# zerohd4869/MM-DFN

Measured on AMD Instinct MI355X. Metric: utterances/sec (fwd+bwd), IEMOCAP-shaped batch, higher is better.
Workload: dtype f32; 1 GPU; cfg2 (BASELINE configs[1]): B=16 dialogues/GPU, L=110, dims 100/100/512, 2 GCN layers, P=2, dropout 0.50; utterances_per_gpu=1760, parallelism=dp1

## Files before the change

mm_dfn_amd/csrc/gemm_tn.hip:

```cpp
#include "mmdfn_internal.h"
#include "../../include/mmdfn_hip.h"
#include <stdlib.h>
#include <algorithm>
#include <stdint.h>

namespace {

constexpr int BR = 32;
constexpr int TM = 64, TN = 64;
constexpr int TNW = 112;
constexpr int LDA = TM + 4;
constexpr int LDB = TN + 4;
constexpr int BS_FLOATS = 32 * (TNW + 4);

inline bool tn_wide(int N) {
    const double e64 = (double)N / (64.0 * ((N + 63) / 64)), e112 = (double)N / (112.0 * ((N + 111) / 112));
    return e112 > e64 + 0.02;
}

template <bool WIDE>
__device__ __forceinline__ void gemm_tn_body(float (*As)[BR * LDA], float* Bs0, const float* __restrict__ A,
                                             const float* __restrict__ B, float* __restrict__ part,
                                             float* __restrict__ colpart, int R, int M, int N, int lda, int ldb,
                                             int rows_per_split, int bshift, int tile, int split) {
// ... 405 lines not shown
            const int64_t idx = t >> 3;
            const bool live = idx < total + M && (idx < total || cs != nullptr);
            const float* src = idx < total ? part + idx : colpart + (idx - total);
            const int64_t sstride = idx < total ? total : M;
            float s = 0.f;
            if (live) {
                int k = sub;
                for (; k + 56 < splits; k += 64) {
                    float v[8];
#pragma unroll
                    for (int e = 0; e < 8; ++e) v[e] = src[(int64_t)(k + 8 * e) * sstride];
#pragma unroll
                    for (int e = 0; e < 8; ++e) s += v[e];
                }
                for (; k < splits; k += 8) s += src[(int64_t)k * sstride];
            }
            s += __shfl_xor(s, 1, 64);
            s += __shfl_xor(s, 2, 64);
            s += __shfl_xor(s, 4, 64);
            if (live && sub == 0) {
                if (idx < total) {
                    const int m = (int)(idx / N);
                    float* dst = C + (int64_t)m * ldc + (idx - (int64_t)m * N);
                    *dst = acc ? *dst + s : s;
                } else {
                    const int m = (int)(idx - total);
                    cs[m] = acc ? cs[m] + s : s;
                    if (cs2 != nullptr) cs2[m] = acc ? cs2[m] + s : s;
                }
            }
        }
        return;
    }
    for (int64_t idx = (blockIdx.x - oq.blk_prefix[p]) * (int64_t)blockDim.x + threadIdx.x; idx < total + M; idx += stride) {
        if (idx < total) {
            float s = 0.f;
            int k = 0;
            for (; k + 8 <= splits; k += 8) {
                float v[8];
#pragma unroll
                for (int e = 0; e < 8; ++e) v[e] = part[(int64_t)(k + e) * total + idx];
#pragma unroll
                for (int e = 0; e < 8; ++e) s += v[e];
            }
            for (; k < splits; ++k) s += part[(int64_t)k * total + idx];
            const int m = (int)(idx / N);
            float* dst = C + (int64_t)m * ldc + (idx - (int64_t)m * N);
            *dst = acc ? *dst + s : s;
        } else if (cs != nullptr) {
            const int m = (int)(idx - total);
            float s = 0.f;
#pragma unroll 8
            for (int k = 0; k < splits; ++k) s += colpart[(int64_t)k * M + m];
            cs[m] = acc ? cs[m] + s : s;
            if (cs2 != nullptr) cs2[m] = acc ? cs2[m] + s : s;
        }
    }
}

}

static int tn_splits_for(int R, int M, int N, int rows_target) {
#ifdef MMDFN_TUNING
    if (const char* e = getenv("MMDFN_TN_SPLITS")) {
        const int v = atoi(e);
        if (v > 0) return v;
// ... 150 lines not shown
}
static int tall_eff_splits(int R, int M, const TallPlan& plan, int* rps_out) {
    const int target = M > 128 ? plan.rows7 : plan.rows2;
    int splits = (R + target - 1) / (target > 0 ? target : 1);
    if (splits < 1) splits = 1;
    const int rps = ((R + splits - 1) / splits + TBR - 1) / TBR * TBR;
    if (rps_out) *rps_out = rps;
    return (R + rps - 1) / rps;
}

static int batch_eff_splits(int R, int M, int N, int rows_target, int* rps_out) {
    int splits = tn_splits_for(R, M, N, 1000);
    if (rows_target > 1000) {
        splits = (R + rows_target - 1) / rows_target;
        if (splits < 1) splits = 1;
    }
    const int rps = ((R + splits - 1) / splits + BR - 1) / BR * BR;
    if (rps_out) *rps_out = rps;
    return (R + rps - 1) / rps;
}

#ifdef MMDFN_TUNING
static bool tns_enabled() { const char* e = getenv("MMDFN_TN_SPLIT"); return !e || atoi(e) != 0; }
#else
constexpr bool tns_enabled() { return true; }
#endif
static bool tns_wide(int N) {
#ifdef MMDFN_TUNING
    if (const char* e = getenv("MMDFN_TNS_WIDE")) { if (atoi(e) == 0) return false; }
#endif
    const int nn = (N + MMDFN_TNS_TN - 1) / MMDFN_TNS_TN, nw = (N + 2 * MMDFN_TNS_TN - 1) / (2 * MMDFN_TNS_TN);
    return 3 * nw < 2 * nn;
}
static int tns_tiles(int M, int N, int* nblocks, int* wide = nullptr) {
    const bool w = tns_wide(N);
    const int bw = w ? 2 * MMDFN_TNS_TN : MMDFN_TNS_TN;
    const int nb = (N + bw - 1) / bw;
    if (nblocks) *nblocks = nb;
    if (wide) *wide = w ? 1 : 0;
    return ((M + MMDFN_TNS_TM - 1) / MMDFN_TNS_TM) * nb;
}
static int tns_rows_target(int nseg, const int* R, const int* out, int nout, const int* M, const int* N, bool riders = false) {
    double units = 0.0;
    for (int s = 0; s < nseg; ++s) {
        const int o = out[s];
        if (o < 0 || o >= nout) continue;
        int wd = 0;
        const int tiles = tns_tiles(M[o], N[o], nullptr, &wd);
        units += (wd ? 1.5 : 1.0) * tiles * R[s];
    }
    double wgs = 384.0;
    if (riders) wgs = 160.0;
#ifdef MMDFN_TUNING
    if (const char* e = getenv("MMDFN_TNS_WGS")) wgs = atof(e);
    if (riders) { if (const char* e = getenv("MMDFN_RIDER_WGS")) wgs = atof(e); }
#endif
    int rt = (int)(units / wgs);
    rt = rt < 256 ? 256 : (rt > 4096 ? 4096 : rt);
    return rt;
}
static int tns_eff_splits(int R, int rows_target, int* rps_out) {
    int splits = 8 * ((R + 4 * rows_target) / (8 * rows_target));
    if (splits < 8) splits = 8;
    const int max_s = (R + 2 * MMDFN_TNS_BK - 1) / (2 * MMDFN_TNS_BK);
    if (splits > max_s) splits = max_s;
    if (splits < 1) splits = 1;
    const int rps = ((R + splits - 1) / splits + MMDFN_TNS_BK - 1) / MMDFN_TNS_BK * MMDFN_TNS_BK;
    if (rps_out) *rps_out = rps;
    return (R + rps - 1) / rps;
}

extern "C" int64_t mmdfn_gemm_tn_batch_workspace(int nseg, const int* R, const int* out, int nout, const int* M,
                                                 const int* N) {
    int64_t total = 0;
    const TallPlan plan = tall_plan(nseg, R, out, nout, M, N);
    const int rt = batch_rows_target(nseg, R, out, nout, M, N, plan.on);
    const int rt_split = tns_rows_target(nseg, R, out, nout, M, N);
    for (int s = 0; s < nseg; ++s) {
        const int o = out[s];
        if (o < 0 || o >= nout) return -1;
        int eff = batch_eff_splits(R[s], M[o], N[o], rt, nullptr);
        if (plan.on && tn_tall_shape1(R[s], M[o], N[o])) eff = std::max(eff, tall_eff_splits(R[s], M[o], plan, nullptr));
        eff = std::max(eff, tns_eff_splits(R[s], rt_split, nullptr));
        total += (int64_t)eff * ((int64_t)M[o] * N[o] + M[o]);
    }
    return total;
}

struct TnExt {
    int n;
    const float* const* part;
    const float* const* colpart;
    float* const* C;
    float* const* colsum;
    const int *M, *N, *ldc, *splits, *accumulate;
};
// ... 149 lines not shown
        std::stable_sort(ord, ord + nseg, [&](int a, int b) { return wg_len(a) > wg_len(b); });
        TnSplitSegs tq;
        tq.n = nseg;
        tq.wg_prefix[0] = 0;
        for (int k = 0; k < nseg; ++k) {
            const int s = ord[k], o = out[s];
            int nb = 1, wd = 0;
            const int tiles = tns_tiles(M[o], N[o], &nb, &wd);
            tq.wide[k] = wd;
            tq.A[k] = A[s]; tq.B[k] = B[s];
            tq.part[k] = part_base[o] + (int64_t)used[o] * M[o] * N[o];
            tq.colpart[k] = (oq.colsum[o] != nullptr) ? col_base[o] + (int64_t)used[o] * M[o] : nullptr;
            used[o] += seg_eff[s];
            tq.R[k] = R[s]; tq.lda[k] = lda[s]; tq.ldb[k] = ldb[s]; tq.bshift[k] = bshift ? bshift[s] : 0;
            tq.rows_per_split[k] = seg_rps[s]; tq.splits[k] = seg_eff[s]; tq.tiles[k] = tiles; tq.nblocks[k] = nb;
            tq.M[k] = M[o]; tq.N[k] = N[o];
            tq.wg_prefix[k + 1] = tq.wg_prefix[k] + tiles * 8 * ((seg_eff[s] + 7) / 8);
        }
        for (int k = nseg; k < MMDFN_TNS_MAXSEG; ++k) {
            tq.A[k] = tq.B[k] = nullptr; tq.part[k] = tq.colpart[k] = nullptr;
            tq.R[k] = tq.lda[k] = tq.ldb[k] = tq.bshift[k] = tq.rows_per_split[k] = tq.splits[k] = tq.tiles[k] = tq.nblocks[k] = 0;
            tq.M[k] = tq.N[k] = 0; tq.wide[k] = 0;
            tq.wg_prefix[k + 1] = tq.wg_prefix[nseg];
        }
        if (stage && riders != nullptr && nseg <= MMDFN_RIDER_MAXSEG && !riders->rider.valid) {
            RiderPlan& p = riders->rider;
            p.tq = tq;
            std::copy(outs, outs + nout, p.outs);
            p.nout = nout;
            p.valid = true;
            return 0;
        }
        if (int e = mmdfn_launch_gemm_tn_split(tq, st)) return e;
        hipLaunchKernelGGL(gemm_tn_batch_reduce_kernel, dim3(oq.blk_prefix[ntot]), dim3(256), 0, st, oq);
        MMDFN_CHECK_LAUNCH();
        return 0;
    }
    const bool use_wide = !tn_no_wide();
    int order[TN_MAXSEG], no = 0, ntall = 0;
    for (int pass = 0; pass < 3; ++pass)
        for (int s = 0; s < nseg; ++s) {
            const int kind = !seg_tall[s] ? 2 : (tall_kind(M[out[s]]) == 7 ? 0 : 1);
            if (kind != pass) continue;
            order[no++] = s;
            if (seg_tall[s]) ++ntall;
        }
    size_t tall_lds = ntall > 0 ? (size_t)(2 * BR * LDA + 2 * BS_FLOATS) * sizeof(float) : 0;
    sq.n = nseg;
    sq.wg_prefix[0] = 0;
    for (int k = 0; k < nseg; ++k) {
        const int s = order[k];
        const int o = out[s];
        const bool wide = !seg_tall[s] && use_wide && tn_wide(N[o]);
        const int tnw = wide ? TNW : TN;
        const int tiles = seg_tall[s] ? tall_blocks(N[o]) : ((M[o] + TM - 1) / TM) * ((N[o] + tnw - 1) / tnw);
        sq.wide[k] = seg_tall[s] ? tall_block_width(N[o]) : (wide ? 1 : 0);
        sq.A[k] = A[s]; sq.B[k] = B[s];
        sq.part[k] = part_base[o] + (int64_t)used[o] * M[o] * N[o];
        sq.colpart[k] = (oq.colsum[o] != nullptr) ? col_base[o] + (int64_t)used[o] * M[o] : nullptr;
        used[o] += seg_eff[s];
        sq.R[k] = R[s]; sq.lda[k] = lda[s]; sq.ldb[k] = ldb[s]; sq.bshift[k] = bshift ? bshift[s] : 0;
        sq.rows_per_split[k] = seg_rps[s]; sq.tiles[k] = tiles; sq.M[k] = M[o]; sq.N[k] = N[o];
        sq.wg_prefix[k + 1] = sq.wg_prefix[k] + tiles * seg_eff[s];
        if (seg_tall[s]) {
            const int bw = tall_block_width(N[o]);
            const size_t need = 2 * (size_t)(((TBR * M[o] * 4 + 1023) & ~1023) + ((TBR * bw * 4 + 1023) & ~1023)) + 1024;
// ... 89 lines not shown
```

mm_dfn_amd/csrc/gemm_tn_split.hip:

```cpp
#include "gemm_tn_split_body.h"
#include <stdlib.h>


namespace {

using namespace tnsb;

template <int ABL>
__global__ __launch_bounds__(512, 2) void gemm_tn_split_kernel(const TnSplitSegs sq, float* __restrict__ trace) {
    extern __shared__ __attribute__((aligned(16))) unsigned char tns_smem[];
    tns_block<ABL>(sq, (int)blockIdx.x, tns_smem, trace);
}

}

int mmdfn_launch_gemm_tn_split(const TnSplitSegs& sq, hipStream_t s) {
    void (*kern)(const TnSplitSegs, float*) = gemm_tn_split_kernel<0>;
    float* trace = nullptr;
#ifdef MMDFN_TUNING
    if (const char* e = getenv("MMDFN_TRACE_PTR")) trace = reinterpret_cast<float*>(strtoull(e, nullptr, 0));
    if (const char* e = getenv("MMDFN_TNS_ABL")) {
        switch (atoi(e)) {
            case 1: kern = gemm_tn_split_kernel<1>; break;
            case 2: kern = gemm_tn_split_kernel<2>; break;
            case 4: kern = gemm_tn_split_kernel<4>; break;
            case 7: kern = gemm_tn_split_kernel<7>; break;
            case 8: kern = gemm_tn_split_kernel<8>; break;
            case 15: kern = gemm_tn_split_kernel<15>; break;
            case 16: kern = gemm_tn_split_kernel<16>; break;
            default: break;
        }
    }
#endif
    if (int e = mmdfn_allow_big_lds(kern)) return e;
    hipLaunchKernelGGL(kern, dim3(sq.wg_prefix[sq.n]), dim3(512), LDS_B, s, sq, trace);
    MMDFN_CHECK_LAUNCH();
    return 0;
}
```

mm_dfn_amd/csrc/gemm_tn_split_body.h:

```cpp
#pragma once
#include "mmdfn_internal.h"
#include <type_traits>

namespace tnsb {

typedef __bf16 bf16x8 __attribute__((ext_vector_type(8)));
typedef uint32_t u32x4 __attribute__((ext_vector_type(4)));
typedef uint32_t u32x2 __attribute__((ext_vector_type(2)));
typedef short s16x4 __attribute__((ext_vector_type(4)));
#define LDS_AS(T, p) ((__attribute__((address_space(3))) T*)(p))

constexpr int SK = MMDFN_TNS_BK;
constexpr int TSM = MMDFN_TNS_TM;
constexpr int TSN = MMDFN_TNS_TN;
constexpr int NCT = TSN / 16;
constexpr int ROWB = 288;
constexpr int PLANE_B = SK * ROWB;
constexpr int IMG_B = 3 * PLANE_B;
constexpr int STAGE_B = 2 * IMG_B;
constexpr int LDS_B = 2 * STAGE_B;

__device__ __forceinline__ float as_f(uint32_t u) { return __builtin_bit_cast(float, u); }
__device__ __forceinline__ uint32_t as_u(float f) { return __builtin_bit_cast(uint32_t, f); }

__device__ __forceinline__ void cut4(float4 v, uint32_t himask, u32x2& p1, u32x2& p2, u32x2& p3) {
    float x0 = v.x, x1 = v.y, x2 = v.z, x3 = v.w;
    p1 = u32x2{__builtin_amdgcn_perm(as_u(x1), as_u(x0), 0x07060302u), __builtin_amdgcn_perm(as_u(x3), as_u(x2), 0x07060302u)};
    x0 -= as_f(as_u(x0) & himask); x1 -= as_f(as_u(x1) & himask); x2 -= as_f(as_u(x2) & himask); x3 -= as_f(as_u(x3) & himask);
    p2 = u32x2{__builtin_amdgcn_perm(as_u(x1), as_u(x0), 0x07060302u), __builtin_amdgcn_perm(as_u(x3), as_u(x2), 0x07060302u)};
    x0 -= as_f(as_u(x0) & himask); x1 -= as_f(as_u(x1) & himask); x2 -= as_f(as_u(x2) & himask); x3 -= as_f(as_u(x3) & himask);
    p3 = u32x2{__builtin_amdgcn_perm(as_u(x1), as_u(x0), 0x07060302u), __builtin_amdgcn_perm(as_u(x3), as_u(x2), 0x07060302u)};
}

__device__ __forceinline__ u32x4 tr_frag(uint32_t addr) {
    const s16x4 lo = __builtin_amdgcn_ds_read_tr16_b64_v4i16(LDS_AS(s16x4, (uintptr_t)addr));
    const s16x4 hi = __builtin_amdgcn_ds_read_tr16_b64_v4i16(LDS_AS(s16x4, (uintptr_t)(addr + 16 * ROWB)));
    const u32x2 l2 = __builtin_bit_cast(u32x2, lo), h2 = __builtin_bit_cast(u32x2, hi);
    return u32x4{l2.x, l2.y, h2.x, h2.y};
}

__device__ __forceinline__ f32x4 mfma16(u32x4 a, u32x4 b, f32x4 c) {
    return __builtin_amdgcn_mfma_f32_16x16x32_bf16(__builtin_bit_cast(bf16x8, a), __builtin_bit_cast(bf16x8, b), c, 0, 0, 0);
}

constexpr int WTN = 2 * MMDFN_TNS_TN;
constexpr int ROWB_W = 544;
constexpr int PLANE_W = SK * ROWB_W;
constexpr int IMG_W = 3 * PLANE_W;
static_assert(IMG_B + IMG_W <= LDS_B, "the wide form's single stage fits the narrow form's LDS");

__device__ __forceinline__ u32x4 tr_frag_w(uint32_t addr) {
    const s16x4 lo = __builtin_amdgcn_ds_read_tr16_b64_v4i16(LDS_AS(s16x4, (uintptr_t)addr));
    const s16x4 hi = __builtin_amdgcn_ds_read_tr16_b64_v4i16(LDS_AS(s16x4, (uintptr_t)(addr + 16 * ROWB_W)));
    const u32x2 l2 = __builtin_bit_cast(u32x2, lo), h2 = __builtin_bit_cast(u32x2, hi);
    return u32x4{l2.x, l2.y, h2.x, h2.y};
}

template <class SQ>
__device__ __forceinline__ void tns_wide_body(const SQ& sq, const int p, const int local, unsigned char* smem) {
    const int round = (local >> 3) / sq.tiles[p];
    const int tile = (local >> 3) - round * sq.tiles[p];
    const int split = 8 * round + (local & 7);
    if (split >= sq.splits[p]) return;
    const int nbn = sq.nblocks[p];
    const int bm = tile / nbn, bn = tile - bm * nbn;
    const int R = sq.R[p], M = sq.M[p], N = sq.N[p], lda = sq.lda[p], ldb = sq.ldb[p], bshift = sq.bshift[p];
    const float* __restrict__ A = sq.A[p];
    const float* __restrict__ B = sq.B[p];
    const int m0 = bm * TSM, n0 = bn * WTN;
    const int r_begin = split * sq.rows_per_split[p];
    const int r_end = min(R, r_begin + sq.rows_per_split[p]);
    const int nchunks = (r_end - r_begin + SK - 1) / SK;

    const int tid = threadIdx.x, lane = tid & 63;
    const int wv = __builtin_amdgcn_readfirstlane(tid >> 6);
    const int wr = wv & 3, wc = wv >> 2;
    const int quad = tid & 31, lrow = tid >> 5;
    const int qb = tid & 63, rb = tid >> 6;
    const int mrem = M - (m0 + 32 * wr);
    const int ntm = mrem <= 0 ? 0 : (mrem <= 16 ? 1 : 2);
    float* __restrict__ colpart = (bn == 0) ? sq.colpart[p] : nullptr;

    const int ca = (m0 + 4 * quad < M) ? m0 + 4 * quad : 0;
    const int cb = (qb < WTN / 4 && n0 + 4 * qb < N) ? n0 + 4 * qb : 0;
    const uint32_t lds0 = (uint32_t)(uintptr_t)((__attribute__((address_space(3))) void*)smem);
    const uint32_t wra = lds0 + lrow * ROWB + quad * 8;
    const uint32_t wrb = lds0 + IMG_B + rb * ROWB_W + qb * 8;
    const uint32_t rsel = 4 * (lane >> 4) + ((lane & 15) >> 2);
    const uint32_t rda = lds0 + rsel * ROWB + (lane & 3) * 8 + 64 * wr;
    const uint32_t rdb = lds0 + IMG_B + rsel * ROWB_W + (lane & 3) * 8 + 2 * MMDFN_TNS_TN * wc;
    uint32_t himask;
    asm volatile("s_mov_b32 %0, 0xffff0000" : "=s"(himask));

    f32x4 acc[2][NCT];
#pragma unroll
    for (int i = 0; i < 2; ++i)
#pragma unroll
        for (int j = 0; j < NCT; ++j) acc[i][j] = (f32x4){0.f, 0.f, 0.f, 0.f};
    float4 cs = make_float4(0.f, 0.f, 0.f, 0.f);
    float4 na[2], nb[4];

    auto inside = [&](int c) {
        const int r0 = r_begin + c * SK;
        return c < nchunks && r0 + SK <= r_end && r0 + bshift >= 0 && r0 + SK - 1 + bshift < R;
    };
    uint32_t offa[2], offb[4];
#pragma unroll
    for (int e = 0; e < 2; ++e) offa[e] = (uint32_t)((lrow + 16 * e) * lda + ca) << 2;
#pragma unroll
    for (int e = 0; e < 4; ++e) offb[e] = (uint32_t)((rb + 8 * e) * ldb + cb) << 2;
    auto issue = [&](int c) {
        uint32_t va[2], vb[4];
        if (inside(c)) {
            const int r0 = r_begin + c * SK;
            const uint32_t sa = (uint32_t)(r0 * lda) << 2, sb = (uint32_t)((r0 + bshift) * ldb) << 2;
#pragma unroll
            for (int e = 0; e < 2; ++e) va[e] = sa + offa[e];
#pragma unroll
            for (int e = 0; e < 4; ++e) vb[e] = sb + offb[e];
        } else {
            const int r0 = r_begin + (c < nchunks ? c : nchunks - 1) * SK;
#pragma unroll
            for (int e = 0; e < 2; ++e) {
                const int rc = min(r0 + lrow + 16 * e, r_end - 1);
                va[e] = (__umul24((uint32_t)rc, (uint32_t)lda) + (uint32_t)ca) << 2;
            }
#pragma unroll
            for (int e = 0; e < 4; ++e) {
                const int rc = min(r0 + rb + 8 * e, r_end - 1);
                const int rbc = min(max(rc + bshift, 0), R - 1);
                vb[e] = (__umul24((uint32_t)rbc, (uint32_t)ldb) + (uint32_t)cb) << 2;
            }
        }
#pragma unroll
        for (int e = 0; e < 2; ++e) na[e] = *reinterpret_cast<const float4*>(reinterpret_cast<const char*>(A) + va[e]);
#pragma unroll
        for (int e = 0; e < 4; ++e) nb[e] = *reinterpret_cast<const float4*>(reinterpret_cast<const char*>(B) + vb[e]);
    };
    float4 ta[2], tb[4];
    auto stage_body = [&](auto edge_tag, int c) {
        constexpr bool EDGE = decltype(edge_tag)::value;
        const int r0 = r_begin + c * SK;
#pragma unroll
        for (int e = 0; e < 2; ++e) {
            float4 xa = ta[e];
            if (EDGE) {
                const bool aok = r0 + lrow + 16 * e < r_end;
                xa = make_float4(aok ? xa.x : 0.f, aok ? xa.y : 0.f, aok ? xa.z : 0.f, aok ? xa.w : 0.f);
            }
            if (colpart) { cs.x += xa.x; cs.y += xa.y; cs.z += xa.z; cs.w += xa.w; }
            u32x2 a1, a2, a3;
            cut4(xa, himask, a1, a2, a3);
            const uint32_t d = wra + e * 16 * ROWB;
            *LDS_AS(u32x2, (uintptr_t)d) = a1;
            *LDS_AS(u32x2, (uintptr_t)(d + PLANE_B)) = a2;
            *LDS_AS(u32x2, (uintptr_t)(d + 2 * PLANE_B)) = a3;
        }
#pragma unroll
        for (int e = 0; e < 4; ++e) {
            float4 xb = tb[e];
            if (EDGE) {
                const int r = r0 + rb + 8 * e;
                const bool bok = r < r_end && r + bshift >= 0 && r + bshift < R;
                xb = make_float4(bok ? xb.x : 0.f, bok ? xb.y : 0.f, bok ? xb.z : 0.f, bok ? xb.w : 0.f);
            }
            u32x2 b1, b2, b3;
            cut4(xb, himask, b1, b2, b3);
            const uint32_t d = wrb + e * 8 * ROWB_W;
            *LDS_AS(u32x2, (uintptr_t)d) = b1;
            *LDS_AS(u32x2, (uintptr_t)(d + PLANE_W)) = b2;
            *LDS_AS(u32x2, (uintptr_t)(d + 2 * PLANE_W)) = b3;
        }
    };
    auto stage = [&](int c) {
#pragma unroll
        for (int e = 0; e < 2; ++e) ta[e] = na[e];
#pragma unroll
        for (int e = 0; e < 4; ++e) tb[e] = nb[e];
        __builtin_amdgcn_sched_barrier(0);
        issue(c + 1);
        __builtin_amdgcn_sched_barrier(0);
        if (inside(c)) stage_body(std::false_type{}, c);
        else stage_body(std::true_type{}, c);
    };
    const int ncol = N - (n0 + MMDFN_TNS_TN * wc);
    const int nlive = ncol <= 0 ? 0 : (ncol >= MMDFN_TNS_TN ? NCT : (ncol + 15) / 16);
    auto mma = [&](auto ntm_tag, auto nl_tag) {
        constexpr int NTM = decltype(ntm_tag)::value;
        constexpr int NL = decltype(nl_tag)::value;
        u32x4 af[NTM][3], bf[3][NL];
#pragma unroll
        for (int q = 0; q < 3; ++q)
#pragma unroll
            for (int i = 0; i < NTM; ++i) af[i][q] = tr_frag(rda + q * PLANE_B + 32 * i);
#pragma unroll
        for (int q = 0; q < 3; ++q)
#pragma unroll
            for (int j = 0; j < NL; ++j) bf[q][j] = tr_frag_w(rdb + q * PLANE_W + 32 * j);
#pragma unroll
        for (int pc = 0; pc < 6; ++pc) {
            const int ai = (pc == 0) ? 2 : (pc == 1 || pc == 3) ? 1 : 0;
            const int bi = (pc < 3) ? 0 : (pc < 5) ? 1 : 2;
#pragma unroll
            for (int j = 0; j < NL; ++j)
#pragma unroll
                for (int i = 0; i < NTM; ++i) acc[i][j] = mfma16(af[i][ai], bf[bi][j], acc[i][j]);
        }
    };
    auto mma_nl = [&](auto ntm_tag) {
        switch (nlive) {
            case 7: mma(ntm_tag, std::integral_constant<int, 7>{}); break;
            case 6: mma(ntm_tag, std::integral_constant<int, 6>{}); break;
            case 5: mma(ntm_tag, std::integral_constant<int, 5>{}); break;
            case 4: mma(ntm_tag, std::integral_constant<int, 4>{}); break;
            case 3: mma(ntm_tag, std::integral_constant<int, 3>{}); break;
            case 2: mma(ntm_tag, std::integral_constant<int, 2>{}); break;
            case 1: mma(ntm_tag, std::integral_constant<int, 1>{}); break;
            default: break;
        }
    };

    issue(0);
#pragma unroll 1
    for (int k = 0; k < nchunks; ++k) {
        stage(k);
        __syncthreads();
        if (ntm == 2) mma_nl(std::integral_constant<int, 2>{});
        else if (ntm == 1) mma_nl(std::integral_constant<int, 1>{});
        __syncthreads();
    }
    if (ntm > 0) {
        float* P = sq.part[p] + (int64_t)split * M * N;
        const int fi = lane & 15, g = lane >> 4;
#pragma unroll
        for (int i = 0; i < 2; ++i)
#pragma unroll
            for (int j = 0; j < NCT; ++j) {
                const int n = n0 + MMDFN_TNS_TN * wc + 16 * j + fi;
#pragma unroll
                for (int r = 0; r < 4; ++r) {
                    const int m = m0 + 32 * wr + 16 * i + 4 * g + r;
                    if (m < M && n < N) P[(int64_t)m * N + n] = acc[i][j][r];
                }
            }
    }
    if (colpart) {
        float* red = reinterpret_cast<float*>(smem);
        *reinterpret_cast<float4*>(red + (tid >> 5) * TSM + 4 * quad) = cs;
        __syncthreads();
        if (tid < TSM && m0 + tid < M) {
            float s = 0.f;
#pragma unroll
            for (int k = 0; k < 16; ++k) s += red[k * TSM + tid];
            colpart[(int64_t)split * M + m0 + tid] = s;
        }
    }
}

template <int ABL, class SQ>
__device__ __forceinline__ void tns_block(const SQ& sq, const int bid, unsigned char* tns_smem, float* __restrict__ trace) {
    int p = 0;
    while (p + 1 < sq.n && bid >= sq.wg_prefix[p + 1]) ++p;
    const int local = bid - sq.wg_prefix[p];
    if (sq.wide[p]) {
        if (ABL == 0) tns_wide_body(sq, p, local, tns_smem);
        return;
    }
    const int round = (local >> 3) / sq.tiles[p];
    const int tile = (local >> 3) - round * sq.tiles[p];
    const int split = 8 * round + (local & 7);
    if (split >= sq.splits[p]) return;
    const int nbn = sq.nblocks[p];
    const int bm = tile / nbn, bn = tile - bm * nbn;
    const int R = sq.R[p], M = sq.M[p], N = sq.N[p], lda = sq.lda[p], ldb = sq.ldb[p], bshift = sq.bshift[p];
    const float* __restrict__ A = sq.A[p];
    const float* __restrict__ B = sq.B[p];
    const int m0 = bm * TSM, n0 = bn * TSN;
    const int r_begin = split * sq.rows_per_split[p];
    const int r_end = min(R, r_begin + sq.rows_per_split[p]);
    const int nchunks = (r_end - r_begin + SK - 1) / SK;

    const int tid = threadIdx.x, lane = tid & 63;
    const int wv = __builtin_amdgcn_readfirstlane(tid >> 6);
    const int grp = wv >> 2, w = wv & 3;
    const int quad = tid & 31, lrow = (tid >> 5) & 7;
    const int mrem = M - (m0 + 32 * w);
    const int ntm = mrem <= 0 ? 0 : (mrem <= 16 ? 1 : 2);
    float* __restrict__ colpart = (bn == 0) ? sq.colpart[p] : nullptr;

    const int ca = (m0 + 4 * quad < M) ? m0 + 4 * quad : 0;
    const int cb = (quad < TSN / 4 && n0 + 4 * quad < N) ? n0 + 4 * quad : 0;
    const uint32_t lds0 = (uint32_t)(uintptr_t)((__attribute__((address_space(3))) void*)tns_smem) + grp * STAGE_B;
    const uint32_t wr = lds0 + lrow * ROWB + quad * 8;
    const uint32_t rd = lds0 + (4 * (lane >> 4) + ((lane & 15) >> 2)) * ROWB + (lane & 3) * 8;
    uint32_t himask;
    asm volatile("s_mov_b32 %0, 0xffff0000" : "=s"(himask));

    f32x4 acc[2][NCT];
// ... 120 lines not shown
            for (int i = 0; i < NTM; ++i)
#pragma unroll
                for (int j = 0; j < NCT; ++j)
                    acc[i][j][0] += as_f(af[i][0].x ^ af[i][1].y ^ af[i][2].z ^ bf[0][j].x ^ bf[1][j].y ^ bf[2][j].z);
            return;
        }
#pragma unroll
        for (int pc = 0; pc < 6; ++pc) {
            const int ai = (pc == 0) ? 2 : (pc == 1 || pc == 3) ? 1 : 0;
            const int bi = (pc < 3) ? 0 : (pc < 5) ? 1 : 2;
#pragma unroll
            for (int j = 0; j < NCT; ++j)
#pragma unroll
                for (int i = 0; i < NTM; ++i) acc[i][j] = mfma16(af[i][ai], bf[bi][j], acc[i][j]);
        }
    };

    issue(grp);
    if (grp == 0) stage(0);
    __syncthreads();
    const long long t_begin = now();
#pragma unroll 1
    for (int k = 0; k < nchunks; ++k) {
        if ((k & 1) == grp) {
            const long long t0 = now();
            if (ntm == 2) mma(std::integral_constant<int, 2>{});
            else if (ntm == 1) mma(std::integral_constant<int, 1>{});
            if (ABL & 16) asm volatile("s_nop 0" ::: "memory");
            tm[3] += now() - t0;
        } else if (k + 1 < nchunks) {
            stage(k + 1);
        }
        const long long t3 = now();
        __syncthreads();
        tm[4] += now() - t3;
    }
    if ((ABL & 16) && trace && (tid == 0 || tid == 256)) {
        float* o = trace + (int64_t)bid * 32 + (tid ? 16 : 0);
        o[0] = (float)tm[0]; o[1] = (float)tm[1]; o[2] = (float)tm[2]; o[3] = (float)tm[3]; o[4] = (float)tm[4];
        o[6] = (float)nchunks; o[7] = (float)(now() - t_begin);
    }
    if (grp == 1 && ntm > 0) {
        float* xch = reinterpret_cast<float*>(tns_smem + (LDS_B - 2 * NCT * 4096)) + (w * 64 + lane) * 4;
#pragma unroll
        for (int i = 0; i < 2; ++i)
#pragma unroll
            for (int j = 0; j < NCT; ++j) *reinterpret_cast<f32x4*>(xch + (i * NCT + j) * 1024) = acc[i][j];
    }
    __syncthreads();
    if (grp == 0 && ntm > 0) {
        const float* xch = reinterpret_cast<const float*>(tns_smem + (LDS_B - 2 * NCT * 4096)) + (w * 64 + lane) * 4;
#pragma unroll
        for (int i = 0; i < 2; ++i)
#pragma unroll
            for (int j = 0; j < NCT; ++j) acc[i][j] += *reinterpret_cast<const f32x4*>(xch + (i * NCT + j) * 1024);
        float* P = sq.part[p] + (int64_t)split * M * N;
        const int fi = lane & 15, g = lane >> 4;
#pragma unroll
        for (int i = 0; i < 2; ++i)
#pragma unroll
            for (int j = 0; j < NCT; ++j) {
                const int n = n0 + 16 * j + fi;
#pragma unroll
                for (int r = 0; r < 4; ++r) {
                    const int m = m0 + 32 * w + 16 * i + 4 * g + r;
                    if (m < M && n < N) P[(int64_t)m * N + n] = acc[i][j][r];
                }
            }
    }
    if (colpart) {
        float* red = reinterpret_cast<float*>(tns_smem);
        *reinterpret_cast<float4*>(red + (tid >> 5) * TSM + 4 * quad) = cs;
        __syncthreads();
        if (tid < TSM && m0 + tid < M) {
            float s = 0.f;
#pragma unroll
            for (int k = 0; k < 16; ++k) s += red[k * TSM + tid];
            colpart[(int64_t)split * M + m0 + tid] = s;
        }
    }
}
}
```

mm_dfn_amd/csrc/gru_mfma.hip:

```cpp
#include "mmdfn_internal.h"
#include "gemm_tn_split_body.h"
#include "keep_flags_body.h"
#include <stdlib.h>

namespace {

constexpr int GH = 100;
typedef __bf16 bf16x8 __attribute__((ext_vector_type(8)));
typedef uint32_t u32x4 __attribute__((ext_vector_type(4)));
typedef uint32_t u32x2 __attribute__((ext_vector_type(2)));
#define LDS_AS(T, p) ((__attribute__((address_space(3))) T*)(p))

constexpr int MS = 16;
constexpr int NWV = 7;
constexpr int NTH = 64 * NWV;
constexpr int HROWB = 272;
constexpr int HPLANE = MS * HROWB;
constexpr int DROWB = 656;
constexpr int DPLANE = MS * DROWB;

__device__ __forceinline__ float as_f(uint32_t u) { return __builtin_bit_cast(float, u); }
__device__ __forceinline__ uint32_t as_u(float f) { return __builtin_bit_cast(uint32_t, f); }

__device__ __forceinline__ void cut4(float x0, float x1, float x2, float x3, u32x2& p1, u32x2& p2, u32x2& p3) {
// ... 387 lines not shown
            u32x2 p1, p2, p3;
            cut4(drp[0], drp[1], drp[2], drp[3], p1, p2, p3);
            *LDS_AS(u32x2, (uintptr_t)wb) = p1;
            *LDS_AS(u32x2, (uintptr_t)(wb + DPLANE)) = p2;
            *LDS_AS(u32x2, (uintptr_t)(wb + 2 * DPLANE)) = p3;
            cut4(dzp[0], dzp[1], dzp[2], dzp[3], p1, p2, p3);
            *LDS_AS(u32x2, (uintptr_t)(wb + 2 * GH)) = p1;
            *LDS_AS(u32x2, (uintptr_t)(wb + 2 * GH + DPLANE)) = p2;
            *LDS_AS(u32x2, (uintptr_t)(wb + 2 * GH + 2 * DPLANE)) = p3;
            cut4(dgn[0], dgn[1], dgn[2], dgn[3], p1, p2, p3);
            *LDS_AS(u32x2, (uintptr_t)(wb + 4 * GH)) = p1;
            *LDS_AS(u32x2, (uintptr_t)(wb + 4 * GH + DPLANE)) = p2;
            *LDS_AS(u32x2, (uintptr_t)(wb + 4 * GH + 2 * DPLANE)) = p3;
        }
        step_barrier();
        if (uok && rok) {
            float* o = dgi + t * gstep;
            *reinterpret_cast<float4*>(o) = make_float4(drp[0], drp[1], drp[2], drp[3]);
            *reinterpret_cast<float4*>(o + GH) = make_float4(dzp[0], dzp[1], dzp[2], dzp[3]);
            *reinterpret_cast<float4*>(o + 2 * GH) = make_float4(dnp[0], dnp[1], dnp[2], dnp[3]);
            float* h = dgh + t * gstep;
            __builtin_nontemporal_store(f32x4{drp[0], drp[1], drp[2], drp[3]}, reinterpret_cast<f32x4*>(h));
            __builtin_nontemporal_store(f32x4{dzp[0], dzp[1], dzp[2], dzp[3]}, reinterpret_cast<f32x4*>(h + GH));
            __builtin_nontemporal_store(f32x4{dgn[0], dgn[1], dgn[2], dgn[3]}, reinterpret_cast<f32x4*>(h + 2 * GH));
        }
    }
}

__global__ __launch_bounds__(BWD_THREADS) void gru_seq_bwd_mfma_kernel(const MfBwd G) {
    extern __shared__ __attribute__((aligned(16))) unsigned char gm_smem[];
    gru_bwd_mfma_body(G, (int)blockIdx.x, (int)blockIdx.y, gm_smem);
}

static_assert(BWD_THREADS == 512 && BWD_LDS >= tnsb::LDS_B, "the rider tiles run in this launch's workgroup shape");
__global__ __launch_bounds__(BWD_THREADS) void gru_seq_bwd_mfma_riders_kernel(const MfBwd G, const TnRiderSegs rq, const int nslots,
                                                                               const int ngru8) {
    extern __shared__ __attribute__((aligned(16))) unsigned char gm_smem[];
    const int bid = (int)blockIdx.x;
    if (bid < 2 * nslots) {
        gru_bwd_mfma_body(G, bid % nslots, bid / nslots, gm_smem);
    } else if (bid >= ngru8) {
        tnsb::tns_block<0>(rq, bid - ngru8, gm_smem, nullptr);
    }
}

}

int mmdfn_launch_gru_fwd_mfma(const GruForm& f, int ngroups, const float* const* gi, const float* const* w_hh,
                              const float* const* b_hh, float* const* y, float* const* gates, const int* rows, const int* T,
                              MmdfnRiders* riders, hipStream_t s) {
    if (ngroups <= 0 || ngroups > MAXG) return -2;
    MfFwd G;
    G.n = ngroups;
    int sl = 0;
    for (int g = 0; g < MAXG; ++g) {
        const bool on = g < ngroups;
        G.gi[g] = on ? gi[g] : nullptr; G.y[g] = on ? y[g] : nullptr; G.gates[g] = on ? gates[g] : nullptr;
        G.w_hh[2 * g] = on ? w_hh[2 * g] : nullptr; G.w_hh[2 * g + 1] = on ? w_hh[2 * g + 1] : nullptr;
        G.b_hh[2 * g] = on ? b_hh[2 * g] : nullptr; G.b_hh[2 * g + 1] = on ? b_hh[2 * g + 1] : nullptr;
        G.rows[g] = on ? rows[g] : 0; G.T[g] = on ? T[g] : 0; G.slice0[g] = sl;
        if (on) sl += (rows[g] + MS - 1) / MS;
    }
    G.slice0[MAXG] = sl;
    for (int g = ngroups; g < MAXG; ++g) G.slice0[g] = sl;
    G.abl = 0;
#ifdef MMDFN_TUNING
    if (const char* e = getenv("MMDFN_GRU_MF_ABL")) G.abl = atoi(e);
// ... 7 lines not shown
        hipLaunchKernelGGL(gru_seq_fwd_mfma_flags_kernel, dim3(2 * sl + (int)nr), dim3(FWD_THREADS), FWD_LDS, s, G, J, sl);
        MMDFN_CHECK_LAUNCH();
        return 0;
    }
    if (int e = mmdfn_allow_big_lds(gru_seq_fwd_mfma_kernel)) return e;
    hipLaunchKernelGGL(gru_seq_fwd_mfma_kernel, dim3(sl, 2), dim3(FWD_THREADS), FWD_LDS, s, G);
    MMDFN_CHECK_LAUNCH();
    return 0;
}

int mmdfn_launch_gru_bwd_mfma(const GruForm& f, int ngroups, const float* const* dy, const float* const* y,
                              const float* const* gates, const float* const* w_hh, float* const* dgi, float* const* dgh,
                              const int* rows, const int* T, MmdfnRiders* riders, hipStream_t s) {
    if (ngroups <= 0 || ngroups > MAXG) return -2;
    MfBwd G;
    G.n = ngroups;
    int sl = 0;
    for (int g = 0; g < MAXG; ++g) {
        const bool on = g < ngroups;
        G.dy[g] = on ? dy[g] : nullptr; G.y[g] = on ? y[g] : nullptr; G.gates[g] = on ? gates[g] : nullptr;
        G.w_hh[2 * g] = on ? w_hh[2 * g] : nullptr; G.w_hh[2 * g + 1] = on ? w_hh[2 * g + 1] : nullptr;
        G.dgi[g] = on ? dgi[g] : nullptr; G.dgh[g] = on ? dgh[g] : nullptr;
        G.rows[g] = on ? rows[g] : 0; G.T[g] = on ? T[g] : 0; G.slice0[g] = sl;
        if (on) sl += (rows[g] + MS - 1) / MS;
    }
    G.slice0[MAXG] = sl;
    for (int g = ngroups; g < MAXG; ++g) G.slice0[g] = sl;
    G.abl = 0;
    if (f.idle_cus > 0 && riders != nullptr && riders->rider.valid && riders->rider.tq.n <= MMDFN_RIDER_MAXSEG) {
        const TnSplitSegs& rp = riders->rider.tq;
        const TnRiderSegs rq = mmdfn_rider_table(rp);
        const int ngru8 = (2 * sl + 7) & ~7;
        if (int e = mmdfn_allow_big_lds(gru_seq_bwd_mfma_riders_kernel)) return e;
        hipLaunchKernelGGL(gru_seq_bwd_mfma_riders_kernel, dim3(ngru8 + rp.wg_prefix[rp.n]), dim3(BWD_THREADS), BWD_LDS, s, G, rq, sl,
                           ngru8);
        MMDFN_CHECK_LAUNCH();
        return mmdfn_riders_launched(riders, s);
    }
    if (int e = mmdfn_allow_big_lds(gru_seq_bwd_mfma_kernel)) return e;
    hipLaunchKernelGGL(gru_seq_bwd_mfma_kernel, dim3(sl, 2), dim3(BWD_THREADS), BWD_LDS, s, G);
    MMDFN_CHECK_LAUNCH();
    return 0;
}
```

Measured before the change: 2.152 million utterances/s.

## Double-buffer wide split-K TN GEMM stages and vectorize the split reduction

The wide form of the split-K TN GEMM now keeps two LDS stages and alternates warp groups between staging the next chunk and running MFMA on the current one, so global loads and LDS writes overlap the products with one barrier per chunk. LDS_B grows to two wide stages, which also raises the rider launch's dynamic LDS. The split-partials reduce kernel gains a float4 path when N, ldc and pointers are 16-byte aligned. The change also adds tuning-only ablation templates and env knobs. The larger LDS footprint keeps one workgroup per CU and may affect the rider kernel co-running with the GRU backward.

```diff
diff --git a/mm_dfn_amd/csrc/gemm_tn.hip b/mm_dfn_amd/csrc/gemm_tn.hip
--- a/mm_dfn_amd/csrc/gemm_tn.hip
+++ b/mm_dfn_amd/csrc/gemm_tn.hip
@@ -461,6 +461,40 @@
         }
         return;
     }
+    if (((N | ldc) & 3) == 0 && ((((uintptr_t)part | (uintptr_t)C) & 15) == 0)) {
+        const int64_t tot4 = total >> 2;
+        for (int64_t idx = (blockIdx.x - oq.blk_prefix[p]) * (int64_t)blockDim.x + threadIdx.x; idx < tot4 + M; idx += stride) {
+            if (idx < tot4) {
+                const float4* src = reinterpret_cast<const float4*>(part) + idx;
+                float4 s = make_float4(0.f, 0.f, 0.f, 0.f);
+                int k = 0;
+                for (; k + 8 <= splits; k += 8) {
+                    float4 v[8];
+#pragma unroll
+                    for (int e = 0; e < 8; ++e) v[e] = src[(int64_t)(k + e) * tot4];
+#pragma unroll
+                    for (int e = 0; e < 8; ++e) { s.x += v[e].x; s.y += v[e].y; s.z += v[e].z; s.w += v[e].w; }
+                }
+                for (; k < splits; ++k) {
+                    const float4 v = src[(int64_t)k * tot4];
+                    s.x += v.x; s.y += v.y; s.z += v.z; s.w += v.w;
+                }
+                const int64_t e0 = idx << 2;
+                const int m = (int)(e0 / N);
+                float4* dst = reinterpret_cast<float4*>(C + (int64_t)m * ldc + (e0 - (int64_t)m * N));
+                if (acc) { const float4 c = *dst; s.x = c.x + s.x; s.y = c.y + s.y; s.z = c.z + s.z; s.w = c.w + s.w; }
+                *dst = s;
+            } else if (cs != nullptr) {
+                const int m = (int)(idx - tot4);
+                float s = 0.f;
+#pragma unroll 8
+                for (int k = 0; k < splits; ++k) s += colpart[(int64_t)k * M + m];
+                cs[m] = acc ? cs[m] + s : s;
+                if (cs2 != nullptr) cs2[m] = acc ? cs2[m] + s : s;
+            }
+        }
+        return;
+    }
     for (int64_t idx = (blockIdx.x - oq.blk_prefix[p]) * (int64_t)blockDim.x + threadIdx.x; idx < total + M; idx += stride) {
         if (idx < total) {
             float s = 0.f;
@@ -677,12 +711,18 @@
     const int nn = (N + MMDFN_TNS_TN - 1) / MMDFN_TNS_TN, nw = (N + 2 * MMDFN_TNS_TN - 1) / (2 * MMDFN_TNS_TN);
     return 3 * nw < 2 * nn;
 }
+static int tns_wide_form() {
+#ifdef MMDFN_TUNING
+    if (const char* e = getenv("MMDFN_TNS_WIDE")) { if (atoi(e) == 2) return 2; }
+#endif
+    return 1;
+}
 static int tns_tiles(int M, int N, int* nblocks, int* wide = nullptr) {
     const bool w = tns_wide(N);
     const int bw = w ? 2 * MMDFN_TNS_TN : MMDFN_TNS_TN;
     const int nb = (N + bw - 1) / bw;
     if (nblocks) *nblocks = nb;
-    if (wide) *wide = w ? 1 : 0;
+    if (wide) *wide = w ? tns_wide_form() : 0;
     return ((M + MMDFN_TNS_TM - 1) / MMDFN_TNS_TM) * nb;
 }
 static int tns_rows_target(int nseg, const int* R, const int* out, int nout, const int* M, const int* N, bool riders = false) {
@@ -705,8 +745,12 @@
     return rt;
 }
 static int tns_eff_splits(int R, int rows_target, int* rps_out) {
-    int splits = 8 * ((R + 4 * rows_target) / (8 * rows_target));
-    if (splits < 8) splits = 8;
+    int unit = 8;
+#ifdef MMDFN_TUNING
+    if (const char* e = getenv("MMDFN_TNS_SPLIT_UNIT")) { if (atoi(e) > 0) unit = atoi(e); }
+#endif
+    int splits = unit * ((R + unit * rows_target / 2) / (unit * rows_target));
+    if (splits < unit) splits = unit;
     const int max_s = (R + 2 * MMDFN_TNS_BK - 1) / (2 * MMDFN_TNS_BK);
     if (splits > max_s) splits = max_s;
     if (splits < 1) splits = 1;
@@ -922,6 +966,9 @@
             return 0;
         }
         if (int e = mmdfn_launch_gemm_tn_split(tq, st)) return e;
+#ifdef MMDFN_TUNING
+        if (const char* e = getenv("MMDFN_TNS_NOREDUCE")) { if (atoi(e) != 0) return 0; }
+#endif
         hipLaunchKernelGGL(gemm_tn_batch_reduce_kernel, dim3(oq.blk_prefix[ntot]), dim3(256), 0, st, oq);
         MMDFN_CHECK_LAUNCH();
         return 0;
diff --git a/mm_dfn_amd/csrc/gemm_tn_split.hip b/mm_dfn_amd/csrc/gemm_tn_split.hip
--- a/mm_dfn_amd/csrc/gemm_tn_split.hip
+++ b/mm_dfn_amd/csrc/gemm_tn_split.hip
@@ -28,6 +28,11 @@
             case 8: kern = gemm_tn_split_kernel<8>; break;
             case 15: kern = gemm_tn_split_kernel<15>; break;
             case 16: kern = gemm_tn_split_kernel<16>; break;
+            case 32: kern = gemm_tn_split_kernel<32>; break;
+            case 64: kern = gemm_tn_split_kernel<64>; break;
+            case 47: kern = gemm_tn_split_kernel<47>; break;
+            case 79: kern = gemm_tn_split_kernel<79>; break;
+            case 111: kern = gemm_tn_split_kernel<111>; break;
             default: break;
         }
     }
diff --git a/mm_dfn_amd/csrc/gemm_tn_split_body.h b/mm_dfn_amd/csrc/gemm_tn_split_body.h
--- a/mm_dfn_amd/csrc/gemm_tn_split_body.h
+++ b/mm_dfn_amd/csrc/gemm_tn_split_body.h
@@ -18,7 +18,7 @@
 constexpr int PLANE_B = SK * ROWB;
 constexpr int IMG_B = 3 * PLANE_B;
 constexpr int STAGE_B = 2 * IMG_B;
-constexpr int LDS_B = 2 * STAGE_B;
+constexpr int LDS_NARROW = 2 * STAGE_B;
 
 __device__ __forceinline__ float as_f(uint32_t u) { return __builtin_bit_cast(float, u); }
 __device__ __forceinline__ uint32_t as_u(float f) { return __builtin_bit_cast(uint32_t, f); }
@@ -47,7 +47,10 @@
 constexpr int ROWB_W = 544;
 constexpr int PLANE_W = SK * ROWB_W;
 constexpr int IMG_W = 3 * PLANE_W;
-static_assert(IMG_B + IMG_W <= LDS_B, "the wide form's single stage fits the narrow form's LDS");
+constexpr int STAGE_W = IMG_B + IMG_W;
+constexpr int LDS_B = 2 * STAGE_W;
+static_assert(LDS_B >= LDS_NARROW && LDS_B <= 156 * 1024, "two wide stages cover the narrow form and fit the opt-in limit");
+static_assert(2 * LDS_B > 160 * 1024, "one workgroup per CU: the rider launches rest on it");
 
 __device__ __forceinline__ u32x4 tr_frag_w(uint32_t addr) {
     const s16x4 lo = __builtin_amdgcn_ds_read_tr16_b64_v4i16(LDS_AS(s16x4, (uintptr_t)addr));
@@ -56,12 +59,14 @@
     return u32x4{l2.x, l2.y, h2.x, h2.y};
 }
 
-template <class SQ>
-__device__ __forceinline__ void tns_wide_body(const SQ& sq, const int p, const int local, unsigned char* smem) {
+template <int ABL, bool TWO, class SQ>
+__device__ __forceinline__ void tns_wide_body(const SQ& sq, const int p, const int local, unsigned char* smem,
+                                              float* __restrict__ stamp) {
     const int round = (local >> 3) / sq.tiles[p];
     const int tile = (local >> 3) - round * sq.tiles[p];
     const int split = 8 * round + (local & 7);
     if (split >= sq.splits[p]) return;
+    if ((ABL & 16) && stamp && threadIdx.x == 0) stamp[15] = TWO ? 2.f : 1.f;
     const int nbn = sq.nblocks[p];
     const int bm = tile / nbn, bn = tile - bm * nbn;
     const int R = sq.R[p], M = sq.M[p], N = sq.N[p], lda = sq.lda[p], ldb = sq.ldb[p], bshift = sq.bshift[p];
@@ -110,6 +115,7 @@
 #pragma unroll
     for (int e = 0; e < 4; ++e) offb[e] = (uint32_t)((rb + 8 * e) * ldb + cb) << 2;
     auto issue = [&](int c) {
+        if (ABL & 8) return;
         uint32_t va[2], vb[4];
         if (inside(c)) {
             const int r0 = r_begin + c * SK;
@@ -138,20 +144,22 @@
         for (int e = 0; e < 4; ++e) nb[e] = *reinterpret_cast<const float4*>(reinterpret_cast<const char*>(B) + vb[e]);
     };
     float4 ta[2], tb[4];
-    auto stage_body = [&](auto edge_tag, int c) {
+    auto stage_body = [&](auto edge_tag, int c, uint32_t so) {
         constexpr bool EDGE = decltype(edge_tag)::value;
         const int r0 = r_begin + c * SK;
 #pragma unroll
         for (int e = 0; e < 2; ++e) {
             float4 xa = ta[e];
+            if (ABL & 8) xa = make_float4(1.f + c, 2.f, 3.f, 4.f);
             if (EDGE) {
                 const bool aok = r0 + lrow + 16 * e < r_end;
                 xa = make_float4(aok ? xa.x : 0.f, aok ? xa.y : 0.f, aok ? xa.z : 0.f, aok ? xa.w : 0.f);
             }
             if (colpart) { cs.x += xa.x; cs.y += xa.y; cs.z += xa.z; cs.w += xa.w; }
             u32x2 a1, a2, a3;
-            cut4(xa, himask, a1, a2, a3);
-            const uint32_t d = wra + e * 16 * ROWB;
+            if (ABL & 1) { a1 = u32x2{as_u(xa.x), as_u(xa.y)}; a2 = u32x2{as_u(xa.z), as_u(xa.w)}; a3 = a1; }
+            else cut4(xa, himask, a1, a2, a3);
+            const uint32_t d = wra + so + e * 16 * ROWB;
             *LDS_AS(u32x2, (uintptr_t)d) = a1;
             *LDS_AS(u32x2, (uintptr_t)(d + PLANE_B)) = a2;
             *LDS_AS(u32x2, (uintptr_t)(d + 2 * PLANE_B)) = a3;
@@ -159,20 +167,22 @@
 #pragma unroll
         for (int e = 0; e < 4; ++e) {
             float4 xb = tb[e];
+            if (ABL & 8) xb = make_float4(4.f, 3.f, 2.f + c, 1.f);
             if (EDGE) {
                 const int r = r0 + rb + 8 * e;
                 const bool bok = r < r_end && r + bshift >= 0 && r + bshift < R;
                 xb = make_float4(bok ? xb.x : 0.f, bok ? xb.y : 0.f, bok ? xb.z : 0.f, bok ? xb.w : 0.f);
             }
             u32x2 b1, b2, b3;
-            cut4(xb, himask, b1, b2, b3);
-            const uint32_t d = wrb + e * 8 * ROWB_W;
+            if (ABL & 1) { b1 = u32x2{as_u(xb.x), as_u(xb.y)}; b2 = u32x2{as_u(xb.z), as_u(xb.w)}; b3 = b1; }
+            else cut4(xb, himask, b1, b2, b3);
+            const uint32_t d = wrb + so + e * 8 * ROWB_W;
             *LDS_AS(u32x2, (uintptr_t)d) = b1;
             *LDS_AS(u32x2, (uintptr_t)(d + PLANE_W)) = b2;
             *LDS_AS(u32x2, (uintptr_t)(d + 2 * PLANE_W)) = b3;
         }
     };
-    auto stage = [&](int c) {
+    auto stage = [&](int c, uint32_t so) {
 #pragma unroll
         for (int e = 0; e < 2; ++e) ta[e] = na[e];
 #pragma unroll
@@ -180,23 +190,41 @@
         __builtin_amdgcn_sched_barrier(0);
         issue(c + 1);
         __builtin_amdgcn_sched_barrier(0);
-        if (inside(c)) stage_body(std::false_type{}, c);
-        else stage_body(std::true_type{}, c);
+        if (inside(c)) stage_body(std::false_type{}, c, so);
+        else stage_body(std::true_type{}, c, so);
     };
     const int ncol = N - (n0 + MMDFN_TNS_TN * wc);
     const int nlive = ncol <= 0 ? 0 : (ncol >= MMDFN_TNS_TN ? NCT : (ncol + 15) / 16);
-    auto mma = [&](auto ntm_tag, auto nl_tag) {
+    auto mma = [&](auto ntm_tag, auto nl_tag, uint32_t so) {
         constexpr int NTM = decltype(ntm_tag)::value;
         constexpr int NL = decltype(nl_tag)::value;
         u32x4 af[NTM][3], bf[3][NL];
-#pragma unroll
-        for (int q = 0; q < 3; ++q)
-#pragma unroll
-            for (int i = 0; i < NTM; ++i) af[i][q] = tr_frag(rda + q * PLANE_B + 32 * i);
-#pragma unroll
-        for (int q = 0; q < 3; ++q)
-#pragma unroll
-            for (int j = 0; j < NL; ++j) bf[q][j] = tr_frag_w(rdb + q * PLANE_W + 32 * j);
+        if (ABL & 4) {
+#pragma unroll
+            for (int q = 0; q < 3; ++q) {
+#pragma unroll
+                for (int i = 0; i < NTM; ++i) af[i][q] = u32x4{(uint32_t)q, 1u, 2u, (uint32_t)i + so};
+#pragma unroll
+                for (int j = 0; j < NL; ++j) bf[q][j] = u32x4{(uint32_t)j, q + 1u, 2u, 3u};
+            }
+        } else {
+#pragma unroll
+            for (int q = 0; q < 3; ++q)
+#pragma unroll
+                for (int i = 0; i < NTM; ++i) af[i][q] = tr_frag(rda + so + q * PLANE_B + 32 * i);
+#pragma unroll
+            for (int q = 0; q < 3; ++q)
+#pragma unroll
+                for (int j = 0; j < NL; ++j) bf[q][j] = tr_frag_w(rdb + so + q * PLANE_W + 32 * j);
+        }
+        if (ABL & 2) {
+#pragma unroll
+            for (int i = 0; i < NTM; ++i)
+#pragma unroll
+                for (int j = 0; j < NL; ++j)
+                    acc[i][j][0] += as_f(af[i][0].x ^ af[i][1].y ^ af[i][2].z ^ bf[0][j].x ^ bf[1][j].y ^ bf[2][j].z);
+            return;
+        }
 #pragma unroll
         for (int pc = 0; pc < 6; ++pc) {
             const int ai = (pc == 0) ? 2 : (pc == 1 || pc == 3) ? 1 : 0;
@@ -207,27 +235,49 @@
                 for (int i = 0; i < NTM; ++i) acc[i][j] = mfma16(af[i][ai], bf[bi][j], acc[i][j]);
         }
     };
-    auto mma_nl = [&](auto ntm_tag) {
+    auto mma_nl = [&](auto ntm_tag, uint32_t so) {
         switch (nlive) {
-            case 7: mma(ntm_tag, std::integral_constant<int, 7>{}); break;
-            case 6: mma(ntm_tag, std::integral_constant<int, 6>{}); break;
-            case 5: mma(ntm_tag, std::integral_constant<int, 5>{}); break;
-            case 4: mma(ntm_tag, std::integral_constant<int, 4>{}); break;
-            case 3: mma(ntm_tag, std::integral_constant<int, 3>{}); break;
-            case 2: mma(ntm_tag, std::integral_constant<int, 2>{}); break;
-            case 1: mma(ntm_tag, std::integral_constant<int, 1>{}); break;
+            case 7: mma(ntm_tag, std::integral_constant<int, 7>{}, so); break;
+            case 6: mma(ntm_tag, std::integral_constant<int, 6>{}, so); break;
+            case 5: mma(ntm_tag, std::integral_constant<int, 5>{}, so); break;
+            case 4: mma(ntm_tag, std::integral_constant<int, 4>{}, so); break;
+            case 3: mma(ntm_tag, std::integral_constant<int, 3>{}, so); break;
+            case 2: mma(ntm_tag, std::integral_constant<int, 2>{}, so); break;
+            case 1: mma(ntm_tag, std::integral_constant<int, 1>{}, so); break;
             default: break;
         }
     };
+    auto products = [&](uint32_t so) {
+        if (ntm == 2) mma_nl(std::integral_constant<int, 2>{}, so);
+        else if (ntm == 1) mma_nl(std::integral_constant<int, 1>{}, so);
+    };
+    auto chunk_barrier = [&]() {
+        if (!(ABL & 32)) __syncthreads();
+    };
 
     issue(0);
+    if (TWO) {
+        stage(0, 0);
+        chunk_barrier();
 #pragma unroll 1
-    for (int k = 0; k < nchunks; ++k) {
-        stage(k);
-        __syncthreads();
-        if (ntm == 2) mma_nl(std::integral_constant<int, 2>{});
-        else if (ntm == 1) mma_nl(std::integral_constant<int, 1>{});
-        __syncthreads();
+        for (int h = 0; h < 2 * nchunks; ++h) {
+            const int k = h >> 1;
+            const uint32_t cur = (k & 1) ? (uint32_t)STAGE_W : 0u;
+            if (((h ^ wc) & 1) == 0) {
+                if (k + 1 < nchunks) stage(k + 1, (uint32_t)STAGE_W - cur);
+            } else {
+                products(cur);
+            }
+            if (h & 1) chunk_barrier();
+        }
+    } else {
+#pragma unroll 1
+        for (int k = 0; k < nchunks; ++k) {
+            stage(k, 0);
+            chunk_barrier();
+            products(0);
+            chunk_barrier();
+        }
     }
     if (ntm > 0) {
         float* P = sq.part[p] + (int64_t)split * M * N;
@@ -240,7 +290,7 @@
 #pragma unroll
                 for (int r = 0; r < 4; ++r) {
                     const int m = m0 + 32 * wr + 16 * i + 4 * g + r;
-                    if (m < M && n < N) P[(int64_t)m * N + n] = acc[i][j][r];
+                    if (m < M && n < N && (!(ABL & 64) || acc[i][j][r] == 1.2345e-30f)) P[(int64_t)m * N + n] = acc[i][j][r];
                 }
             }
     }
@@ -252,7 +302,7 @@
             float s = 0.f;
 #pragma unroll
             for (int k = 0; k < 16; ++k) s += red[k * TSM + tid];
-            colpart[(int64_t)split * M + m0 + tid] = s;
+            if (!(ABL & 64) || s == 1.2345e-30f) colpart[(int64_t)split * M + m0 + tid] = s;
         }
     }
 }
@@ -263,7 +313,13 @@
     while (p + 1 < sq.n && bid >= sq.wg_prefix[p + 1]) ++p;
     const int local = bid - sq.wg_prefix[p];
     if (sq.wide[p]) {
-        if (ABL == 0) tns_wide_body(sq, p, local, tns_smem);
+#ifdef MMDFN_TUNING
+        if (sq.wide[p] == 2) {
+            tns_wide_body<ABL, false>(sq, p, local, tns_smem, trace ? trace + (int64_t)bid * 32 : nullptr);
+            return;
+        }
+#endif
+        tns_wide_body<ABL, true>(sq, p, local, tns_smem, trace ? trace + (int64_t)bid * 32 : nullptr);
         return;
     }
     const int round = (local >> 3) / sq.tiles[p];
@@ -450,7 +506,7 @@
             stage(k + 1);
         }
         const long long t3 = now();
-        __syncthreads();
+        if (!(ABL & 32)) __syncthreads();
         tm[4] += now() - t3;
     }
     if ((ABL & 16) && trace && (tid == 0 || tid == 256)) {
@@ -459,7 +515,7 @@
         o[6] = (float)nchunks; o[7] = (float)(now() - t_begin);
     }
     if (grp == 1 && ntm > 0) {
-        float* xch = reinterpret_cast<float*>(tns_smem + (LDS_B - 2 * NCT * 4096)) + (w * 64 + lane) * 4;
+        float* xch = reinterpret_cast<float*>(tns_smem + (LDS_NARROW - 2 * NCT * 4096)) + (w * 64 + lane) * 4;
 #pragma unroll
         for (int i = 0; i < 2; ++i)
 #pragma unroll
@@ -467,7 +523,7 @@
     }
     __syncthreads();
     if (grp == 0 && ntm > 0) {
-        const float* xch = reinterpret_cast<const float*>(tns_smem + (LDS_B - 2 * NCT * 4096)) + (w * 64 + lane) * 4;
+        const float* xch = reinterpret_cast<const float*>(tns_smem + (LDS_NARROW - 2 * NCT * 4096)) + (w * 64 + lane) * 4;
 #pragma unroll
         for (int i = 0; i < 2; ++i)
 #pragma unroll
@@ -482,7 +538,7 @@
 #pragma unroll
                 for (int r = 0; r < 4; ++r) {
                     const int m = m0 + 32 * w + 16 * i + 4 * g + r;
-                    if (m < M && n < N) P[(int64_t)m * N + n] = acc[i][j][r];
+                    if (m < M && n < N && (!(ABL & 64) || acc[i][j][r] == 1.2345e-30f)) P[(int64_t)m * N + n] = acc[i][j][r];
                 }
             }
     }
@@ -494,8 +550,8 @@
             float s = 0.f;
 #pragma unroll
             for (int k = 0; k < 16; ++k) s += red[k * TSM + tid];
-            colpart[(int64_t)split * M + m0 + tid] = s;
-        }
-    }
-}
-}
+            if (!(ABL & 64) || s == 1.2345e-30f) colpart[(int64_t)split * M + m0 + tid] = s;
+        }
+    }
+}
+}
diff --git a/mm_dfn_amd/csrc/gru_mfma.hip b/mm_dfn_amd/csrc/gru_mfma.hip
--- a/mm_dfn_amd/csrc/gru_mfma.hip
+++ b/mm_dfn_amd/csrc/gru_mfma.hip
@@ -443,7 +443,9 @@
     gru_bwd_mfma_body(G, (int)blockIdx.x, (int)blockIdx.y, gm_smem);
 }
 
-static_assert(BWD_THREADS == 512 && BWD_LDS >= tnsb::LDS_B, "the rider tiles run in this launch's workgroup shape");
+static_assert(BWD_THREADS == 512, "the rider tiles run in this launch's workgroup shape");
+constexpr int RIDER_LDS = BWD_LDS > tnsb::LDS_B ? BWD_LDS : tnsb::LDS_B;
+static_assert(RIDER_LDS <= 156 * 1024 && 2 * RIDER_LDS > 160 * 1024, "within the opt-in limit, one workgroup per CU");
 __global__ __launch_bounds__(BWD_THREADS) void gru_seq_bwd_mfma_riders_kernel(const MfBwd G, const TnRiderSegs rq, const int nslots,
                                                                                const int ngru8) {
     extern __shared__ __attribute__((aligned(16))) unsigned char gm_smem[];
@@ -517,7 +519,7 @@
         const TnRiderSegs rq = mmdfn_rider_table(rp);
         const int ngru8 = (2 * sl + 7) & ~7;
         if (int e = mmdfn_allow_big_lds(gru_seq_bwd_mfma_riders_kernel)) return e;
-        hipLaunchKernelGGL(gru_seq_bwd_mfma_riders_kernel, dim3(ngru8 + rp.wg_prefix[rp.n]), dim3(BWD_THREADS), BWD_LDS, s, G, rq, sl,
+        hipLaunchKernelGGL(gru_seq_bwd_mfma_riders_kernel, dim3(ngru8 + rp.wg_prefix[rp.n]), dim3(BWD_THREADS), RIDER_LDS, s, G, rq, sl,
                            ngru8);
         MMDFN_CHECK_LAUNCH();
         return mmdfn_riders_launched(riders, s);
```

Result: no change. 2.170 million utterances/s (median of 6 runs) (+0.8%).
